# MechaCritter/Python-Visual-Similarity

Hardware: AMD Instinct MI355X
Metric: images/sec encoded + top-k retrieved, VLAD K256 RootSIFT (higher is better)
Workload: dtype f32

## Files before the change

include/pvsim.h:

```cpp
#ifndef PVSIM_H
#define PVSIM_H

#include <stddef.h>
#include <stdint.h>

#ifdef __cplusplus
extern "C" {
#endif

#define PVS_VERSION 103

typedef enum {
  PVS_OK = 0,
  PVS_ERR_INVALID = 1,
  PVS_ERR_NO_DEVICE = 2,
  PVS_ERR_OOM = 3,
  PVS_ERR_UNSUPPORTED = 4,
  PVS_ERR_DIM = 5,
  PVS_ERR_CAPACITY = 6
} pvs_status;

typedef enum {
  PVS_DESC_F32 = 0,
  PVS_DESC_F32_ROOTSIFT = 1,
  PVS_DESC_U8_ROOTSIFT = 2
} pvs_desc_kind;

typedef enum {
  PVS_OPT_ASSIGN_PREFILTER = 0,
  PVS_OPT_VLAD_PATH = 1,
  PVS_OPT_TOPK_SELECT_ONLY = 2,
  PVS_OPT_AGG_VARIANT = 3,
  PVS_OPT_FISHER_SCALE = 4,
  PVS_OPT_COUNT_ = 5
} pvs_option;

typedef struct pvs_ctx pvs_ctx;
typedef struct pvs_codebook pvs_codebook;
typedef struct pvs_gmm pvs_gmm;
typedef struct pvs_pca pvs_pca;
typedef struct pvs_comm pvs_comm;

typedef struct {
  double power_norm_weight;
  double norm_order;
  double epsilon;
} pvs_norm_params;

int pvs_version(void);
// ... 129 lines not shown
  PVS_DSIFT_F32_RAW = 2,
  PVS_DSIFT_F32_QUANT = 3
} pvs_dsift_out;
int pvs_dsift_count(int H, int W, int step, const int32_t* sizes, int n_sizes, int64_t* count);
int pvs_dsift_frames(int H, int W, int step, const int32_t* sizes, int n_sizes, float* frames , int64_t capacity);
int pvs_dsift_dev(pvs_ctx* ctx, const void* d_pixels, int pixel_kind, const int32_t* h_hw, const int64_t* h_pix_offsets,
                  int64_t n_images, int step, const int32_t* sizes, int n_sizes, double contrast_threshold, int out_kind,
                  void* d_out, int64_t out_rows, int64_t* d_row_offsets);

int pvs_sift_workspace(int H, int W, int n_octave_layers, int upsample, size_t* bytes, int64_t* max_rows);
int pvs_sift_dev(pvs_ctx* ctx, const void* d_pixels, int pixel_kind, const int32_t* h_hw, const int64_t* h_pix_offsets,
                 int64_t n_images, int nfeatures, int n_octave_layers, double contrast_threshold, double edge_threshold, double sigma,
                 int upsample, int out_kind, void* d_rows, int64_t capacity_rows, float* d_frames ,
                 int64_t* d_row_offsets, int64_t* h_total_rows);

#define PVS_TIMER_SLOTS 8
int pvs_timers_enable(pvs_ctx* ctx, int on);
int pvs_timers_reset(pvs_ctx* ctx);
int pvs_timers_read(pvs_ctx* ctx, int which, double* total_ms, int64_t* launches);

#ifdef __cplusplus
}
#endif
#endif
```

python-visual-similarity_amd/csrc/api.hip:

```cpp
#include <algorithm>
#include <cmath>
#include <limits>
#include <memory>

#include "common.hpp"

namespace pvs {

static thread_local char g_err[512] = "";

void set_error(const char* fmt, ...) {
  va_list ap;
  va_start(ap, fmt);
  vsnprintf(g_err, sizeof(g_err), fmt, ap);
  va_end(ap);
}

int ws_reserve(pvs_ctx* ctx, int which, size_t bytes, void** out) {
  if (bytes == 0) bytes = 16;
  if (ctx->ws_bytes[which] < bytes) {
    if (ctx->ws[which]) {
      PVS_HIP(hipStreamSynchronize(ctx->stream));
      PVS_HIP(hipFree(ctx->ws[which]));
      ctx->ws[which] = nullptr;
// ... 176 lines not shown

PVS_EXPORT void* pvs_stream(pvs_ctx* ctx) { return ctx ? static_cast<void*>(ctx->stream) : nullptr; }

PVS_EXPORT int pvs_device_name(pvs_ctx* ctx, char* buf, size_t buflen) {
  PVS_NEED(ctx, "ctx");
  PVS_NEED(buf, "buf");
  hipDeviceProp_t prop;
  PVS_HIP(hipGetDeviceProperties(&prop, ctx->device));
  snprintf(buf, buflen, "%s (%s, %d CUs)", prop.name, prop.gcnArchName, prop.multiProcessorCount);
  return PVS_OK;
}

PVS_EXPORT int pvs_set_option(pvs_ctx* ctx, int option, int value) {
  PVS_NEED(ctx, "ctx");
  if (option < 0 || option >= PVS_OPT_COUNT_) PVS_FAIL(PVS_ERR_INVALID, "unknown option %d", option);
  const int hi = option == PVS_OPT_ASSIGN_PREFILTER ? 4 : (option == PVS_OPT_VLAD_PATH || option == PVS_OPT_TOPK_SELECT_ONLY) ? 3 : ((option == PVS_OPT_AGG_VARIANT || option == PVS_OPT_FISHER_SCALE) ? 2 : 1);
  if (value < 0 || value > hi) PVS_FAIL(PVS_ERR_INVALID, "option %d: value %d out of range 0..%d", option, value, hi);
  ctx->opt[option] = value;
  return PVS_OK;
}
PVS_EXPORT int pvs_get_option(pvs_ctx* ctx, int option, int* value) {
  PVS_NEED(ctx, "ctx");
  PVS_NEED(value, "value");
  if (option < 0 || option >= PVS_OPT_COUNT_) PVS_FAIL(PVS_ERR_INVALID, "unknown option %d", option);
  *value = ctx->opt[option];
  return PVS_OK;
}

PVS_EXPORT int pvs_malloc(pvs_ctx* ctx, size_t bytes, void** dptr) {
  PVS_NEED(ctx, "ctx");
  PVS_NEED(dptr, "dptr");
// ... 594 lines not shown
      const int64_t cn = std::min(NC, N - c0);
      const float* iq = d_inv_q ? d_inv_q + q0 : nullptr;
      const float* idb = d_inv_db ? d_inv_db + c0 : nullptr;
      if (f16)
        PVS_TRY(launch_cosine_f16(ctx, q + (size_t)q0 * L * esz, qn, db + (size_t)c0 * L * esz, cn, L, iq, idb, panel, cn));
      else
        PVS_TRY(launch_cosine_f32(ctx, reinterpret_cast<const float*>(q) + q0 * L, qn,
                                  reinterpret_cast<const float*>(db) + c0 * L, cn, L, iq, idb, panel, cn));
      PVS_TRY(launch_topk(ctx, panel, qn, cn, cn, k, col_offset + c0, (merge || c0 > 0) ? 1 : 0, d_idx + q0 * k,
                          d_val + q0 * k));
    }
  }
  return PVS_OK;
}

PVS_EXPORT int pvs_cosine_topk_dev(pvs_ctx* ctx, const float* d_Q, int64_t nq, const float* d_DB, int64_t N, int64_t L,
                                   const float* d_inv_q, const float* d_inv_db, int k, int64_t col_offset, int merge,
                                   int64_t* d_idx, float* d_val) {
  return cosine_topk_impl(ctx, d_Q, nq, d_DB, N, L, false, d_inv_q, d_inv_db, k, col_offset, merge, d_idx, d_val);
}

namespace pvs {
int cosine_topk_exact(pvs_ctx* ctx, const float* d_Q, int64_t nq, const float* d_DB, int64_t N, int64_t L, const float* d_inv_q,
                      const float* d_inv_db, int k, int64_t* d_idx, float* d_val) {
  return cosine_topk_impl(ctx, d_Q, nq, d_DB, N, L, false, d_inv_q, d_inv_db, k, 0, 0, d_idx, d_val);
}
}

PVS_EXPORT int pvs_cosine_topk_filtered_dev(pvs_ctx* ctx, const float* d_Q, int64_t nq, const float* d_DB, int64_t N, int64_t L,
                                            const float* d_inv_q, const float* d_inv_db, int k, int64_t* d_idx, float* d_val,
                                            int64_t* h_stats) {
  PVS_NEED(ctx, "ctx");
  if (h_stats) h_stats[0] = h_stats[1] = h_stats[2] = h_stats[3] = 0;
  if (nq <= 0) return PVS_OK;
  PVS_NEED(d_Q, "Q");
  PVS_NEED(d_idx, "idx");
  PVS_NEED(d_val, "val");
  PVS_HIP(hipSetDevice(ctx->device));
  if (N > 0 && d_DB != nullptr) {
    const int rc = launch_cosine_topk_filtered(ctx, d_Q, nq, d_DB, N, L, d_inv_q, d_inv_db, k, 0, d_idx, d_val, h_stats);
    if (rc != PVS_ERR_UNSUPPORTED) return rc;
    if (h_stats) h_stats[0] = h_stats[1] = h_stats[2] = h_stats[3] = 0;
  }
  return cosine_topk_impl(ctx, d_Q, nq, d_DB, N, L, false, d_inv_q, d_inv_db, k, 0, 0, d_idx, d_val);
}

PVS_EXPORT int pvs_cosine_topk_f16_dev(pvs_ctx* ctx, const void* d_Q16, int64_t nq, const void* d_DB16, int64_t N,
                                       int64_t L, const float* d_inv_q, const float* d_inv_db, int k, int64_t col_offset,
                                       int merge, int64_t* d_idx, float* d_val) {
  return cosine_topk_impl(ctx, d_Q16, nq, d_DB16, N, L, true, d_inv_q, d_inv_db, k, col_offset, merge, d_idx, d_val);
}

PVS_EXPORT int pvs_f32_to_f16_dev(pvs_ctx* ctx, const float* d_src, int64_t n, void* d_dst) {
  PVS_NEED(ctx, "ctx");
  if (n <= 0) return PVS_OK;
// ... 32 lines not shown
  char* d_s = nullptr;
  PVS_TRY(ws_reserve(ctx, 0, q_bytes + (same ? 0 : db_bytes), reinterpret_cast<void**>(&d_in)));
  const size_t nrm = ((size_t)(nq + N) * 4 + 255) / 256 * 256, idxb = ((size_t)nq * k * 8 + 255) / 256 * 256;
  PVS_TRY(ws_reserve(ctx, 1, nrm + idxb + (size_t)nq * k * 4, reinterpret_cast<void**>(&d_s)));
  float* dq = reinterpret_cast<float*>(d_in);
  float* ddb = same ? dq : reinterpret_cast<float*>(d_in + q_bytes);
  PVS_HIP(hipMemcpyAsync(dq, Q, (size_t)nq * L * 4, hipMemcpyHostToDevice, ctx->stream));
  if (!same) PVS_HIP(hipMemcpyAsync(ddb, DB, (size_t)N * L * 4, hipMemcpyHostToDevice, ctx->stream));
  float* invq = reinterpret_cast<float*>(d_s);
  float* invd = invq + nq;
  int64_t* d_idx = reinterpret_cast<int64_t*>(d_s + nrm);
  float* d_val = reinterpret_cast<float*>(d_s + nrm + idxb);
  PVS_TRY(launch_row_inv_norms(ctx, dq, nq, L, invq));
  PVS_TRY(launch_row_inv_norms(ctx, ddb, N, L, invd));
  const float* invd_use = same ? invq : invd;
  if (nq >= 512) PVS_TRY(pvs_cosine_topk_filtered_dev(ctx, dq, nq, ddb, N, L, invq, invd_use, k, d_idx, d_val, nullptr));
  else PVS_TRY(pvs_cosine_topk_dev(ctx, dq, nq, ddb, N, L, invq, invd_use, k, 0, 0, d_idx, d_val));
  PVS_HIP(hipMemcpyAsync(out_idx, d_idx, (size_t)nq * k * 8, hipMemcpyDeviceToHost, ctx->stream));
  PVS_HIP(hipMemcpyAsync(out_val, d_val, (size_t)nq * k * 4, hipMemcpyDeviceToHost, ctx->stream));
  PVS_HIP(hipStreamSynchronize(ctx->stream));
  return PVS_OK;
}


PVS_EXPORT int pvs_row_inv_norms_f64_dev(pvs_ctx* ctx, const double* d_x, int64_t rows, int64_t L, double* d_inv) {
  PVS_NEED(ctx, "ctx");
  if (rows <= 0) return PVS_OK;
  PVS_NEED(d_x, "x");
  PVS_NEED(d_inv, "inv");
  PVS_HIP(hipSetDevice(ctx->device));
  return launch_row_inv_norms_f64(ctx, d_x, rows, L, d_inv);
}
// ... 311 lines not shown
```

python-visual-similarity_amd/csrc/common.hpp:

```cpp
#pragma once
#include <hip/hip_runtime.h>

#include <cmath>
#include <cstdarg>
#include <cstdint>
#include <cstdio>
#include <cstring>
#include <map>
#include <vector>

#include "../../include/pvsim.h"
#include "../../include/pvsim_diag.h"

#define PVS_EXPORT extern "C" __attribute__((visibility("default")))

namespace pvs {

void set_error(const char* fmt, ...);

#define PVS_FAIL(code, ...)        \
  do {                             \
    ::pvs::set_error(__VA_ARGS__); \
    return (code);                 \
  } while (0)
// ... 4 lines not shown
    if (e__ != hipSuccess) {                                                             \
      ::pvs::set_error("%s failed: %s (%s:%d)", #expr, hipGetErrorString(e__), __FILE__, \
                       __LINE__);                                                        \
      return e__ == hipErrorOutOfMemory ? PVS_ERR_OOM : PVS_ERR_NO_DEVICE;               \
    }                                                                                    \
  } while (0)

#define PVS_TRY(expr)                 \
  do {                                \
    int s__ = (expr);                 \
    if (s__ != PVS_OK) return s__;    \
  } while (0)

constexpr int WAVE = 64;

enum TimerSlot { T_ASSIGN = 0, T_AGGREGATE = 1, T_GEMM = 2, T_TOPK = 3, T_FPOST = 4, T_FMOM = 5, T_MISC = 6, T_RESCORE = 7 };

struct TimerRec {
  hipEvent_t a, b;
  int slot;
};

}

struct pvs_ctx {
  int device = 0;
  hipStream_t stream = nullptr;
  bool owns_stream = false;
  int num_cu = 256;
  static constexpr int NWS = 13;
  void* ws[NWS] = {};
  size_t ws_bytes[NWS] = {};
  struct GemmPlanSlot {
    int key[4] = {-1, -1, -1, -1};
    int n_main = 0, n_tail = 0, splitk = 1;
    void* d_tiles = nullptr;
    size_t cap = 0;
  } gemm_plan[5];
  std::map<const void*, int> lds_attr;
  int opt[PVS_OPT_COUNT_] = {1, 0, 0, 0, 0};
  unsigned int* d_queue = nullptr;
  unsigned long long* d_fused_stamps = nullptr;
  bool timers_on = false;
  std::vector<pvs::TimerRec> pending;
  std::vector<hipEvent_t> event_pool;
  std::multimap<size_t, void*> block_cache;
  std::map<void*, size_t> block_size;
  size_t block_cache_bytes = 0;
  void* h_stage = nullptr;
  size_t h_stage_bytes = 0;
  static constexpr int DSIFT_RING = 4;
  void* dsift_h[DSIFT_RING] = {};
  size_t dsift_h_bytes[DSIFT_RING] = {};
  hipEvent_t dsift_ev[DSIFT_RING] = {};
  int dsift_next = 0;
// ... 96 lines not shown
                          const int64_t* d_offsets, int64_t n_images, const int32_t* d_labels,
                          const pvs_norm_params& prm, float* d_out, float* d_inv_norm, bool raw = false,
                          const float2* rowstat = nullptr, int64_t total_hint = 0);
bool vlad_fused_eligible(const pvs_codebook* cb, const void* d_desc, int kind, int ld, const float* d_out);
int launch_vlad_fused(pvs_ctx* ctx, const pvs_codebook* cb, const void* d_desc, int kind, int ld, const int64_t* d_offsets,
                      int64_t n_images, const pvs_norm_params& prm, float* d_out, int32_t* d_labels, float* d_inv_norm, bool raw = false);
int launch_row_inv_norms(pvs_ctx* ctx, const float* d_x, int64_t rows, int64_t L, float* d_inv);
int launch_cosine_f32(pvs_ctx* ctx, const float* A, int64_t M, const float* B, int64_t N, int64_t L,
                      const float* inva, const float* invb, float* out, int64_t ldo);
int launch_cosine_f32_dual(pvs_ctx* ctx, const float* A, int64_t M, const float* B, int64_t N, int64_t L, const float* inva,
                           const float* invb, float* out, int64_t ldo, float* out_t, int64_t ldt);
int launch_cosine_f16(pvs_ctx* ctx, const void* A, int64_t M, const void* B, int64_t N, int64_t L, const float* inva,
                      const float* invb, float* out, int64_t ldo);
int launch_f32_to_f16(pvs_ctx* ctx, const float* src, int64_t n, void* dst);
int launch_cosine_f16_bounded(pvs_ctx* ctx, const void* A, int64_t M, const void* B, int64_t N, int64_t L, const float* inva,
                              const float* invb, float* out, int64_t ldo);
int cosine_topk_exact(pvs_ctx* ctx, const float* d_Q, int64_t nq, const float* d_DB, int64_t N, int64_t L, const float* d_inv_q,
                      const float* d_inv_db, int k, int64_t* d_idx, float* d_val);
int launch_cosine_topk_filtered(pvs_ctx* ctx, const float* Q, int64_t nq, const float* DB, int64_t N, int64_t L,
                                const float* invq, const float* invdb, int k, int64_t col_offset, int64_t* d_idx, float* d_val,
                                int64_t* h_stats);
int launch_cosine_f64(pvs_ctx* ctx, const double* A, int64_t M, const double* B, int64_t N, int64_t L, double* out);
int launch_row_inv_norms_f64(pvs_ctx* ctx, const double* d_x, int64_t rows, int64_t L, double* d_inv);
int launch_cosine_f64_dev(pvs_ctx* ctx, const double* A, int64_t M, const double* B, int64_t N, int64_t L, const double* inva,
                          const double* invb, double* out, int64_t ldo);
bool cosine_dense_rows_eligible(const float* Q, const float* DB, int64_t nq, int64_t L);
int launch_cosine_dense_rows(pvs_ctx* ctx, const float* Q, int64_t nq, const float* DB, int64_t N, int64_t L, const float* invq,
                             const float* invdb, float* scores, int64_t ld);
int launch_topk(pvs_ctx* ctx, const float* scores, int64_t nq, int64_t ncols, int64_t ld, int k,
                int64_t col_offset, int merge, int64_t* d_idx, float* d_val);
int launch_topk_merge(pvs_ctx* ctx, const int64_t* idx_lists, const float* val_lists, int n_lists, int64_t nq,
                      int k, int64_t* d_idx, float* d_val);
int launch_rank_f64(pvs_ctx* ctx, const double* scores, int64_t nq, int64_t ncols, int64_t ld, int k, int64_t* d_idx, double* d_val);
int launch_pca(pvs_ctx* ctx, const pvs_pca* p, const void* d_desc, int kind, int64_t total, float* d_out);
int launch_gmm_posterior(pvs_ctx* ctx, const pvs_gmm* g, const void* d_desc, int kind, int ld, int64_t total,
                         double* d_resp);
// ... 19 lines not shown
```

python-visual-similarity_amd/csrc/cosine.hip:

```cpp
#include <algorithm>
#include <type_traits>

#include "common.hpp"
#include "gemm_mfma.hpp"
#include "gemm_f64.hpp"
#include "gemm_f16_8ph.hpp"
#include "gemm_f16_2lvl.hpp"

namespace pvs {

__device__ __attribute__((aligned(16))) float g_zero16[4] = {0.f, 0.f, 0.f, 0.f};

__global__ __launch_bounds__(256) void row_inv_norms_kernel(const float* __restrict__ x, int64_t rows, int64_t L,
                                                            float* __restrict__ inv, int vec) {
  const int lane = threadIdx.x & 63;
  const int64_t row = (int64_t)blockIdx.x * 4 + (threadIdx.x >> 6);
  if (row >= rows) return;
  const float* p = x + row * L;
  float s0 = 0.f, s1 = 0.f, s2 = 0.f, s3 = 0.f;
  if (vec) {
    const float4* p4 = reinterpret_cast<const float4*>(p);
    for (int64_t i = lane; i < (L >> 2); i += 64) {
      const float4 v = p4[i];
      s0 = fmaf(v.x, v.x, s0); s1 = fmaf(v.y, v.y, s1); s2 = fmaf(v.z, v.z, s2); s3 = fmaf(v.w, v.w, s3);
// ... 15 lines not shown
  PVS_HIP(hipGetLastError());
  return PVS_OK;
}

using GemmMain = GemmCfg<128, 128, 2, 2, 2, false>;
using GemmHalf = GemmCfg<256, 256, 2, 4, 2, true>;
using GemmPre = GemmCfg<128, 128, 2, 2, 2, true>;
template <int MODEL> struct GemmModel;
template <> struct GemmModel<0> { using Cfg = GemmMain; static constexpr bool F16 = false, TWO = true; static constexpr int BM = 128, WN = 2, PER_CU = 2; };
template <> struct GemmModel<1> { using Cfg = GemmHalf; static constexpr bool F16 = true, TWO = false; static constexpr int BM = 256, WN = 4, PER_CU = 1; };
template <> struct GemmModel<2> { using Cfg = GemmPre; static constexpr bool F16 = true, TWO = true; static constexpr int BM = 128, WN = 2, PER_CU = 2; };

using GemmPlan = pvs_ctx::GemmPlanSlot;

static int build_plan(pvs_ctx* ctx, int which, int tiles_m, int tiles_n, bool symm, int slots, GemmPlan** out) {
  GemmPlan& P = ctx->gemm_plan[which];
  const int key[4] = {tiles_m, tiles_n, symm ? 1 : 0, slots};
  if (memcmp(P.key, key, sizeof(key)) != 0) {
    std::vector<GemmTile> t;
    if (symm) {
      const int TS = (tiles_m + 7) / 8;
      for (int si = 0; si < TS; ++si)
        for (int sj = si; sj < TS; ++sj)
          for (int w = 0; w < 64; ++w) {
            const int tm = si * 8 + (w & 7), tn = sj * 8 + (w >> 3);
            if (tm < tiles_m && tn < tiles_m && tn >= tm) t.push_back({tm, tn});
          }
    } else {
      for (int g0 = 0; g0 < tiles_m; g0 += 8) {
        const int gsz = std::min(8, tiles_m - g0);
        for (int tn = 0; tn < tiles_n; ++tn)
          for (int dm = 0; dm < gsz; ++dm) t.push_back({g0 + dm, tn});
// ... 149 lines not shown
  PVS_HIP(hipGetLastError());
  return PVS_OK;
}

int launch_cosine_f16(pvs_ctx* ctx, const void* A, int64_t M, const void* B, int64_t N, int64_t L, const float* inva,
                      const float* invb, float* out, int64_t ldo) {
  if (M <= 0 || N <= 0) return PVS_OK;
  if (L <= 0 || L % 8 != 0 || reinterpret_cast<uintptr_t>(A) % 16 || reinterpret_cast<uintptr_t>(B) % 16)
    PVS_FAIL(PVS_ERR_UNSUPPORTED, "fp16 cosine needs 16-B aligned rows (L %% 8 == 0), got L = %lld", (long long)L);
  if (L > (int64_t)8 * 1024 * 1024) PVS_FAIL(PVS_ERR_UNSUPPORTED, "fp16 cosine: L too large");
  ScopedTimer tm(ctx, T_GEMM);
  return cosine_mfma<1>(ctx, A, M, B, N, L, inva, invb, out, ldo);
}

int launch_cosine_f16_bounded(pvs_ctx* ctx, const void* A, int64_t M, const void* B, int64_t N, int64_t L, const float* inva,
                              const float* invb, float* out, int64_t ldo) {
  if (M <= 0 || N <= 0) return PVS_OK;
  if (L <= 0 || L % 8 != 0 || reinterpret_cast<uintptr_t>(A) % 16 || reinterpret_cast<uintptr_t>(B) % 16)
    PVS_FAIL(PVS_ERR_UNSUPPORTED, "fp16 cosine needs 16-B aligned rows (L %% 8 == 0), got L = %lld", (long long)L);
  ScopedTimer tm(ctx, T_GEMM);
  constexpr int64_t SEG = 32768;
  const char* a = static_cast<const char*>(A);
  const char* b = static_cast<const char*>(B);
  for (int64_t k0 = 0; k0 < L; k0 += SEG)
    PVS_TRY(cosine_mfma<2>(ctx, a + k0 * 2, M, A == B ? a + k0 * 2 : b + k0 * 2, N, std::min(SEG, L - k0), inva, invb, out, ldo, nullptr, 0, L,
                           k0 > 0 ? 1 : 0));
  return PVS_OK;
}

template <typename T>
__global__ __launch_bounds__(256) void cosine_gemm_generic_kernel(const T* __restrict__ A, int64_t M,
                                                                  const T* __restrict__ B, int64_t N, int64_t L,
                                                                  const T* __restrict__ inva,
                                                                  const T* __restrict__ invb, T* __restrict__ out,
                                                                  int64_t ldo) {
// ... 155 lines not shown
```

python-visual-similarity_amd/csrc/filter.hip:

```cpp
#include <algorithm>
#include <cmath>
#include <vector>

#include "common.hpp"

namespace pvs {

constexpr int FLT_PASS = 16;
constexpr int FLT_SK = 32;
constexpr int FLT_THREADS = FLT_PASS * 32;

static double filter_eps(int64_t L) {
  return 9.77e-4 * (1.0 + 1.0 / 4096.0) + (1088.0 + (double)L / 1024.0 + 2.0 * (double)((L + 32767) / 32768)) * 1.1920929e-7 +
         2.98e-8 * std::sqrt((double)L);
}

__global__ __launch_bounds__(256) void filter_rows_to_f16_kernel(const float* __restrict__ x, int64_t rows, int64_t L,
                                                                 const float* __restrict__ inv_in, _Float16* __restrict__ out,
                                                                 float* __restrict__ inv_out, unsigned long long* __restrict__ stats) {
  __shared__ float red[4];
  __shared__ int bad[4];
  const int64_t row = blockIdx.x;
  const float4* xr = reinterpret_cast<const float4*>(x + row * L);
  const int64_t n4 = L / 4;
// ... 31 lines not shown
    inv_out[row] = (inv_in ? inv_in[row] : 1.f) * ldexpf(1.f, -sh);
    if (nf) atomicAdd(&stats[0], 1ull);
  }
}

__global__ __launch_bounds__(256) void filter_collect_kernel(const float* __restrict__ S, int64_t nq, int64_t ncols, int64_t ld,
                                                             const int64_t* __restrict__ aidx, const float* __restrict__ aval,
                                                             int k, float margin, int cap, int64_t col_offset, int first,
                                                             int64_t* __restrict__ cand_idx, int* __restrict__ count,
                                                             unsigned long long* __restrict__ stats) {
  const int lane = threadIdx.x & 63;
  const int64_t q = (int64_t)blockIdx.x * 4 + (threadIdx.x >> 6);
  if (q >= nq) return;
  const bool full = aidx[q * k + k - 1] >= 0;
  const float thr = full ? aval[q * k + k - 1] - margin : -INFINITY;
  int base = first ? 0 : count[q];
  const int base0 = base;
  for (int64_t c0 = 0; c0 < ncols; c0 += 64) {
    const int64_t c = c0 + lane;
    const bool pred = c < ncols && S[q * ld + c] >= thr;
    const unsigned long long mask = __ballot(pred);
    if (pred) {
      const int slot = base + __popcll(mask & ((1ull << lane) - 1ull));
      if (slot < cap) cand_idx[((int64_t)(slot / k) * nq + q) * k + slot % k] = col_offset + c;
    }
    base += __popcll(mask);
  }
  if (lane == 0) {
    count[q] = base;
    atomicAdd(&stats[2], (unsigned long long)(base - base0));
    if (base > cap && base0 <= cap) atomicAdd(&stats[1], 1ull);
  }
}

struct RescoreArgs {
  const float* Q;
  const float* DB;
  int64_t nq, L;
  const float* invq;
  const float* invdb;
  const int64_t* cand_idx;
  float* cand_val;
  const int* count;
  int cap, k;
  int64_t col_offset;
// ... 113 lines not shown
int launch_cosine_dense_rows(pvs_ctx* ctx, const float* Q, int64_t nq, const float* DB, int64_t N, int64_t L, const float* invq,
                             const float* invdb, float* scores, int64_t ld) {
  if (!cosine_dense_rows_eligible(Q, DB, nq, L)) PVS_FAIL(PVS_ERR_UNSUPPORTED, "dense row scoring: shape does not qualify");
  if (N <= 0) return PVS_OK;
  const int64_t groups = (N + FLT_PASS - 1) / FLT_PASS;
  if (groups > 0x7fffffffLL) PVS_FAIL(PVS_ERR_UNSUPPORTED, "dense row scoring: too many rows");
  RescoreArgs ra{Q, DB, nq, L, invq, invdb, nullptr, scores, nullptr, 0, 1, 0, N, ld};
  ScopedTimer tm(ctx, T_GEMM);
  hipLaunchKernelGGL(filter_rescore_kernel<true>, dim3((unsigned)groups, (unsigned)nq), dim3(FLT_THREADS), 0, ctx->stream, ra);
  PVS_HIP(hipGetLastError());
  return PVS_OK;
}

int launch_cosine_topk_filtered(pvs_ctx* ctx, const float* Q, int64_t nq, const float* DB, int64_t N, int64_t L,
                                const float* invq, const float* invdb, int k, int64_t col_offset, int64_t* d_idx, float* d_val,
                                int64_t* h_stats) {
  if (col_offset != 0) PVS_FAIL(PVS_ERR_UNSUPPORTED, "filtered top-k: col_offset must be 0");
  if (nq <= 0 || N <= 0) PVS_FAIL(PVS_ERR_UNSUPPORTED, "filtered top-k: empty input");
  if (L > (int64_t)8 * 1024 * 1024) PVS_FAIL(PVS_ERR_UNSUPPORTED, "filtered top-k: rows too long");
  if (L % 8 != 0 || L < 8 || reinterpret_cast<uintptr_t>(Q) % 16 || reinterpret_cast<uintptr_t>(DB) % 16)
    PVS_FAIL(PVS_ERR_UNSUPPORTED, "filtered top-k needs 16-B aligned rows with L %% 8 == 0");
  if (k < 1 || k > 128) PVS_FAIL(PVS_ERR_UNSUPPORTED, "filtered top-k: k <= 128");
  const int64_t NC = std::min<int64_t>(N, 32768);
  const bool multi = N > NC;
  const bool same = (Q == DB) && (nq == N) && (invq == invdb);
  const bool square = same && !multi && (int64_t)nq * N <= ((int64_t)1 << 28);
  const int cap_lists = ((multi ? 16 : 4) * k + (multi ? 128 : 64) + k - 1) / k;
  const int cap = cap_lists * k;
  const int64_t QT = square ? nq : std::min<int64_t>(nq, std::max<int64_t>(256, ((int64_t)1 << 28) / NC));
  const double eps = filter_eps(L);
  const float margin = (float)(2.0 * eps);

  const size_t q16_b = ((size_t)nq * L * 2 + 255) / 256 * 256, db16_b = same ? 0 : ((size_t)N * L * 2 + 255) / 256 * 256;
  char* w5 = nullptr;
  if (ws_reserve(ctx, 5, q16_b + db16_b, reinterpret_cast<void**>(&w5)) != PVS_OK) {
    (void)hipGetLastError();
    PVS_FAIL(PVS_ERR_UNSUPPORTED, "filtered top-k: no device memory for the fp16 copies (%zu bytes)", q16_b + db16_b);
  }
  _Float16* q16 = reinterpret_cast<_Float16*>(w5);
  _Float16* db16 = same ? q16 : reinterpret_cast<_Float16*>(w5 + q16_b);
  auto al = [](size_t b) { return (b + 255) / 256 * 256; };
  const size_t o_invq = 0, o_invd = o_invq + al((size_t)nq * 4), o_stats = o_invd + al((size_t)N * 4),
               o_aidx = o_stats + 256, o_aval = o_aidx + al((size_t)QT * k * 8), o_cidx = o_aval + al((size_t)QT * k * 4),
               o_cval = o_cidx + al((size_t)QT * cap * 8), o_cnt = o_cval + al((size_t)QT * cap * 4), o_end = o_cnt + al((size_t)QT * 4);
  char* w6 = nullptr;
  PVS_TRY(ws_reserve(ctx, 6, o_end, reinterpret_cast<void**>(&w6)));
  float* invq16 = reinterpret_cast<float*>(w6 + o_invq);
  float* invd16 = same ? invq16 : reinterpret_cast<float*>(w6 + o_invd);
  unsigned long long* stats = reinterpret_cast<unsigned long long*>(w6 + o_stats);
  int64_t* aidx = reinterpret_cast<int64_t*>(w6 + o_aidx);
  float* aval = reinterpret_cast<float*>(w6 + o_aval);
  int64_t* cidx = reinterpret_cast<int64_t*>(w6 + o_cidx);
  float* cval = reinterpret_cast<float*>(w6 + o_cval);
  int* cnt = reinterpret_cast<int*>(w6 + o_cnt);
  float* panel = nullptr;
  PVS_TRY(ws_reserve(ctx, 2, (size_t)QT * NC * sizeof(float), reinterpret_cast<void**>(&panel)));
  PVS_HIP(hipMemsetAsync(stats, 0, 32, ctx->stream));

  {
    ScopedTimer tm(ctx, T_MISC);
    hipLaunchKernelGGL(filter_rows_to_f16_kernel, dim3((unsigned)nq), dim3(256), 0, ctx->stream, Q, nq, L, invq, q16, invq16, stats);
    if (!same)
      hipLaunchKernelGGL(filter_rows_to_f16_kernel, dim3((unsigned)N), dim3(256), 0, ctx->stream, DB, N, L, invdb, db16, invd16, stats);
    PVS_HIP(hipGetLastError());
  }
  unsigned long long hs[4] = {0, 0, 0, 0};
  PVS_HIP(hipMemcpyAsync(hs, stats, 8, hipMemcpyDeviceToHost, ctx->stream));
  PVS_HIP(hipStreamSynchronize(ctx->stream));
  if (hs[0]) PVS_FAIL(PVS_ERR_UNSUPPORTED, "filtered top-k: %llu rows hold non-finite values or an extreme dynamic range", hs[0]);

  std::vector<int> h_cnt;
  for (int64_t q0 = 0; q0 < nq; q0 += QT) {
    const int64_t qn = std::min(QT, nq - q0);
    PVS_TRY(ws_reserve(ctx, 2, (size_t)QT * NC * sizeof(float), reinterpret_cast<void**>(&panel)));
    PVS_HIP(hipMemsetAsync(cidx, 0xff, (size_t)qn * cap * 8, ctx->stream));
    for (int64_t c0 = 0; c0 < N; c0 += NC) {
      const int64_t cn = std::min(NC, N - c0);
      PVS_TRY(launch_cosine_f16_bounded(ctx, q16 + q0 * L, qn, db16 + c0 * L, cn, L, invq16 + q0, invd16 + c0, panel, cn));
      PVS_TRY(launch_topk(ctx, panel, qn, cn, cn, k, c0, c0 > 0 ? 1 : 0, aidx, aval));
      ScopedTimer tm(ctx, T_TOPK);
      hipLaunchKernelGGL(filter_collect_kernel, dim3((unsigned)((qn + 3) / 4)), dim3(256), 0, ctx->stream, panel, qn, cn, cn, aidx, aval, k,
                         margin, cap, c0, c0 == 0 ? 1 : 0, cidx, cnt, stats);
    }
    PVS_HIP(hipMemcpyAsync(hs, stats, 24, hipMemcpyDeviceToHost, ctx->stream));
    PVS_HIP(hipStreamSynchronize(ctx->stream));
    if (hs[1] * 10 > (unsigned long long)qn) PVS_FAIL(PVS_ERR_UNSUPPORTED, "filtered top-k: %llu of %lld queries exceed the candidate slots", hs[1], (long long)qn);
    {
      ScopedTimer tm(ctx, T_RESCORE);
      RescoreArgs ra{Q + q0 * L, DB, qn, L, invq ? invq + q0 : nullptr, invdb, cidx, cval, cnt, cap, k, 0};
      hipLaunchKernelGGL(filter_rescore_kernel<false>, dim3((unsigned)qn), dim3(FLT_THREADS), 0, ctx->stream, ra);
    }
    PVS_HIP(hipGetLastError());
    PVS_TRY(launch_topk_merge(ctx, cidx, cval, cap_lists, qn, k, d_idx + q0 * k, d_val + q0 * k));
    PVS_HIP(hipMemcpyAsync(hs, stats, 24, hipMemcpyDeviceToHost, ctx->stream));
    PVS_HIP(hipStreamSynchronize(ctx->stream));
    if (hs[1]) {
      h_cnt.resize((size_t)qn);
      PVS_HIP(hipMemcpy(h_cnt.data(), cnt, (size_t)qn * 4, hipMemcpyDeviceToHost));
      std::vector<int64_t> rows;
      for (int64_t i = 0; i < qn; ++i)
        if (h_cnt[(size_t)i] > cap) rows.push_back(i);
      const int64_t nr = (int64_t)rows.size();
      const int64_t rb = std::max<int64_t>(1, std::min<int64_t>(nr, ((int64_t)1 << 28) / N));
      char* w4 = nullptr;
      const size_t rows_b = al((size_t)nr * 8), g_b = al((size_t)rb * L * 4), gi_b = al((size_t)rb * 4), li_b = al((size_t)rb * k * 8);
      PVS_TRY(ws_reserve(ctx, 3, rows_b + g_b + gi_b + li_b + al((size_t)rb * k * 4), reinterpret_cast<void**>(&w4)));
      int64_t* d_rows = reinterpret_cast<int64_t*>(w4);
      float* gq = reinterpret_cast<float*>(w4 + rows_b);
      float* gi = reinterpret_cast<float*>(w4 + rows_b + g_b);
      int64_t* li = reinterpret_cast<int64_t*>(w4 + rows_b + g_b + gi_b);
      float* lv = reinterpret_cast<float*>(w4 + rows_b + g_b + gi_b + li_b);
      PVS_HIP(hipMemcpyAsync(d_rows, rows.data(), (size_t)nr * 8, hipMemcpyHostToDevice, ctx->stream));
      for (int64_t r0 = 0; r0 < nr; r0 += rb) {
        const int64_t rn = std::min(rb, nr - r0);
        hipLaunchKernelGGL(filter_gather_rows_kernel, dim3((unsigned)rn), dim3(256), 0, ctx->stream, Q + q0 * L, d_rows + r0, L, gq,
                           invq ? invq + q0 : nullptr, gi);
        PVS_HIP(hipGetLastError());
        PVS_TRY(cosine_topk_exact(ctx, gq, rn, DB, N, L, gi, invdb, k, li, lv));
        hipLaunchKernelGGL(filter_scatter_lists_kernel, dim3((unsigned)rn), dim3(64), 0, ctx->stream, li, lv, d_rows + r0, k,
                           d_idx + q0 * k, d_val + q0 * k);
      }
// ... 13 lines not shown
```

python-visual-similarity_amd/pvsim/_ffi.py:

```python
from __future__ import annotations

import ctypes as C
import os
import threading

import numpy as np

from ._errors import CapacityError

_HERE = os.path.dirname(os.path.abspath(__file__))
LIB_PATH = os.environ.get("PVSIM_LIB", os.path.join(_HERE, "libpvsim_hip.so"))

PVS_OK, PVS_ERR_INVALID, PVS_ERR_NO_DEVICE, PVS_ERR_OOM, PVS_ERR_UNSUPPORTED, PVS_ERR_DIM, PVS_ERR_CAPACITY = range(7)
_EXC = {PVS_ERR_INVALID: ValueError, PVS_ERR_NO_DEVICE: RuntimeError, PVS_ERR_OOM: MemoryError,
        PVS_ERR_UNSUPPORTED: NotImplementedError, PVS_ERR_DIM: RuntimeError, PVS_ERR_CAPACITY: CapacityError}

DESC_F32, DESC_F32_ROOTSIFT, DESC_U8_ROOTSIFT = 0, 1, 2
OPT_ASSIGN_PREFILTER, OPT_VLAD_PATH, OPT_TOPK_SELECT_ONLY, OPT_AGG_VARIANT, OPT_FISHER_SCALE = 0, 1, 2, 3, 4
PIX_U8_RGB, PIX_U8_GRAY, PIX_F32_RGB, PIX_F32_GRAY = 0, 1, 2, 3
DSIFT_U8, DSIFT_F32, DSIFT_F32_RAW, DSIFT_F32_QUANT = 0, 1, 2, 3
VLAD_PATH_AUTO, VLAD_PATH_GATHER, VLAD_PATH_STREAM, VLAD_PATH_FUSED = 0, 1, 2, 3
TIMER_NAMES = ("assign", "aggregate", "cosine_gemm", "topk", "fisher_posterior", "fisher_moments", "misc", "rescore")


class NormParams(C.Structure):
    _fields_ = [("power_norm_weight", C.c_double), ("norm_order", C.c_double), ("epsilon", C.c_double)]


_vp, _i64, _int, _sz = C.c_void_p, C.c_int64, C.c_int, C.c_size_t
_pp = C.POINTER(C.c_void_p)
_np = C.POINTER(NormParams)

SIGNATURES = {
    "pvs_version": [],
    "pvs_last_error": [],
    "pvs_device_count": [C.POINTER(C.c_int)],
    "pvs_init": [_int, _vp, _pp],
# ... 151 lines not shown
```

python-visual-similarity_amd/pvsim/distributed.py:

```python
from __future__ import annotations

import ctypes as C
import socket
import struct
import time
from typing import Callable

import numpy as np

__all__ = ["shard_range", "gather_blocks", "mask_padding", "retrieve_sharded", "device_score_block",
           "retrieve_symmetric", "symmetric_local", "symmetric_finish", "DeviceOps", "ShardedVLADIndex",
           "DevArray", "DevicePool", "RcclComm", "new_unique_id", "exchange_unique_id"]

_ITEM = {"float32": 4, "int64": 8, "int32": 4, "float64": 8, "float16": 2, "uint8": 1}


def shard_range(n_total: int, world: int, rank: int) -> tuple[int, int, int]:
    block = (n_total + world - 1) // world
    lo = min(n_total, rank * block)
    return lo, min(n_total, lo + block), block


def exchange_chunks(n_total: int, world: int, n_chunks: int):
    _, _, block = shard_range(n_total, world, 0)
# ... 290 lines not shown

    def score(q, n_q, db, n_db, inv_q, inv_db, k, col_offset, merge, idx, val):
        ctx.cosine_topk_dev(q.data_ptr(), n_q, db.data_ptr(), n_db, q.shape[1], inv_q.data_ptr(), inv_db.data_ptr(),
                            k, col_offset, merge, idx.data_ptr(), val.data_ptr())

    return score


class DeviceOps:

    def __init__(self, ctx, same_stream: bool = False):
        self.ctx = ctx
        self.same_stream = same_stream

    def sym_topk(self, q, n, inv, k, col_offset, idx, val):
        self.ctx.cosine_topk_dev(q.data_ptr(), n, q.data_ptr(), n, q.shape[1], inv.data_ptr(), inv.data_ptr(), k,
                                 col_offset, False, idx.data_ptr(), val.data_ptr())

    def dual(self, a, m, b, n, inv_a, inv_b, panel, panel_t):
        self.ctx.cosine_dual_dev(a.data_ptr(), m, b.data_ptr(), n, a.shape[1], inv_a.data_ptr(), inv_b.data_ptr(),
                                 panel.data_ptr(), n, panel_t.data_ptr(), m)

    def topk(self, scores, nq, ncols, k, col_offset, merge, idx, val):
        self.ctx.topk_dev(scores.data_ptr(), nq, ncols, ncols, k, col_offset, merge, idx.data_ptr(), val.data_ptr())

    def merge(self, idx_lists, val_lists, n_lists, nq, k, idx, val):
        self.ctx.topk_merge_dev(idx_lists.data_ptr(), val_lists.data_ptr(), n_lists, nq, k, idx.data_ptr(), val.data_ptr())

    def sync(self):
        if not self.same_stream:
            self.ctx.sync()

# ... 177 lines not shown
```

Before: 420,700.

## Route default cosine top-k through the filtered fp16 prefilter path with probing

pvs_cosine_topk_dev now defaults to the fp16 prefilter + exact rescore path for large query/database sizes. Before committing to the full run it probes on the first 256 rows. The gemm plan cache becomes two-way so the probe and main tile shapes do not evict each other. A per-tile stats sync moves into the prefilter step, and NaN thresholds now force the overflow path. The aim is to avoid full fp32 GEMM plus top-k for most candidates, at the cost of extra syncs and a fallback risk when candidate slots overflow.

```diff
diff --git a/include/pvsim.h b/include/pvsim.h
--- a/include/pvsim.h
+++ b/include/pvsim.h
@@ -32,7 +32,8 @@
   PVS_OPT_TOPK_SELECT_ONLY = 2,
   PVS_OPT_AGG_VARIANT = 3,
   PVS_OPT_FISHER_SCALE = 4,
-  PVS_OPT_COUNT_ = 5
+  PVS_OPT_TOPK_PATH = 5,
+  PVS_OPT_COUNT_ = 6
 } pvs_option;
 
 typedef struct pvs_ctx pvs_ctx;
@@ -192,7 +193,7 @@
                  int upsample, int out_kind, void* d_rows, int64_t capacity_rows, float* d_frames ,
                  int64_t* d_row_offsets, int64_t* h_total_rows);
 
-#define PVS_TIMER_SLOTS 8
+#define PVS_TIMER_SLOTS 9
 int pvs_timers_enable(pvs_ctx* ctx, int on);
 int pvs_timers_reset(pvs_ctx* ctx);
 int pvs_timers_read(pvs_ctx* ctx, int which, double* total_ms, int64_t* launches);
diff --git a/python-visual-similarity_amd/csrc/api.hip b/python-visual-similarity_amd/csrc/api.hip
--- a/python-visual-similarity_amd/csrc/api.hip
+++ b/python-visual-similarity_amd/csrc/api.hip
@@ -214,7 +214,7 @@
 PVS_EXPORT int pvs_set_option(pvs_ctx* ctx, int option, int value) {
   PVS_NEED(ctx, "ctx");
   if (option < 0 || option >= PVS_OPT_COUNT_) PVS_FAIL(PVS_ERR_INVALID, "unknown option %d", option);
-  const int hi = option == PVS_OPT_ASSIGN_PREFILTER ? 4 : (option == PVS_OPT_VLAD_PATH || option == PVS_OPT_TOPK_SELECT_ONLY) ? 3 : ((option == PVS_OPT_AGG_VARIANT || option == PVS_OPT_FISHER_SCALE) ? 2 : 1);
+  const int hi = option == PVS_OPT_ASSIGN_PREFILTER ? 4 : (option == PVS_OPT_VLAD_PATH || option == PVS_OPT_TOPK_SELECT_ONLY) ? 3 : ((option == PVS_OPT_AGG_VARIANT || option == PVS_OPT_FISHER_SCALE || option == PVS_OPT_TOPK_PATH) ? 2 : 1);
   if (value < 0 || value > hi) PVS_FAIL(PVS_ERR_INVALID, "option %d: value %d out of range 0..%d", option, value, hi);
   ctx->opt[option] = value;
   return PVS_OK;
@@ -839,9 +839,24 @@
   return PVS_OK;
 }
 
+constexpr int64_t TOPK_FILTER_MIN_NQ = 512;
+static int topk_filter_mode(const pvs_ctx* ctx, int64_t nq, int64_t N, int64_t col_offset, int merge) {
+  const int opt = ctx->opt[PVS_OPT_TOPK_PATH];
+  if (opt == 1 || col_offset != 0 || merge != 0 || nq <= 0 || N <= 0) return 0;
+  if (opt == 2) return 2;
+  return (nq >= TOPK_FILTER_MIN_NQ && N >= TOPK_FILTER_MIN_NQ) ? 1 : 0;
+}
+
 PVS_EXPORT int pvs_cosine_topk_dev(pvs_ctx* ctx, const float* d_Q, int64_t nq, const float* d_DB, int64_t N, int64_t L,
                                    const float* d_inv_q, const float* d_inv_db, int k, int64_t col_offset, int merge,
                                    int64_t* d_idx, float* d_val) {
+  PVS_NEED(ctx, "ctx");
+  const int mode = topk_filter_mode(ctx, nq, N, col_offset, merge);
+  if (mode != 0 && d_Q != nullptr && d_DB != nullptr && d_idx != nullptr && d_val != nullptr) {
+    PVS_HIP(hipSetDevice(ctx->device));
+    const int rc = launch_cosine_topk_filtered(ctx, d_Q, nq, d_DB, N, L, d_inv_q, d_inv_db, k, 0, d_idx, d_val, nullptr, mode == 1);
+    if (rc != PVS_ERR_UNSUPPORTED) return rc;
+  }
   return cosine_topk_impl(ctx, d_Q, nq, d_DB, N, L, false, d_inv_q, d_inv_db, k, col_offset, merge, d_idx, d_val);
 }
 
@@ -863,7 +878,7 @@
   PVS_NEED(d_val, "val");
   PVS_HIP(hipSetDevice(ctx->device));
   if (N > 0 && d_DB != nullptr) {
-    const int rc = launch_cosine_topk_filtered(ctx, d_Q, nq, d_DB, N, L, d_inv_q, d_inv_db, k, 0, d_idx, d_val, h_stats);
+    const int rc = launch_cosine_topk_filtered(ctx, d_Q, nq, d_DB, N, L, d_inv_q, d_inv_db, k, 0, d_idx, d_val, h_stats, false);
     if (rc != PVS_ERR_UNSUPPORTED) return rc;
     if (h_stats) h_stats[0] = h_stats[1] = h_stats[2] = h_stats[3] = 0;
   }
@@ -926,8 +941,7 @@
   PVS_TRY(launch_row_inv_norms(ctx, dq, nq, L, invq));
   PVS_TRY(launch_row_inv_norms(ctx, ddb, N, L, invd));
   const float* invd_use = same ? invq : invd;
-  if (nq >= 512) PVS_TRY(pvs_cosine_topk_filtered_dev(ctx, dq, nq, ddb, N, L, invq, invd_use, k, d_idx, d_val, nullptr));
-  else PVS_TRY(pvs_cosine_topk_dev(ctx, dq, nq, ddb, N, L, invq, invd_use, k, 0, 0, d_idx, d_val));
+  PVS_TRY(pvs_cosine_topk_dev(ctx, dq, nq, ddb, N, L, invq, invd_use, k, 0, 0, d_idx, d_val));
   PVS_HIP(hipMemcpyAsync(out_idx, d_idx, (size_t)nq * k * 8, hipMemcpyDeviceToHost, ctx->stream));
   PVS_HIP(hipMemcpyAsync(out_val, d_val, (size_t)nq * k * 4, hipMemcpyDeviceToHost, ctx->stream));
   PVS_HIP(hipStreamSynchronize(ctx->stream));
diff --git a/python-visual-similarity_amd/csrc/common.hpp b/python-visual-similarity_amd/csrc/common.hpp
--- a/python-visual-similarity_amd/csrc/common.hpp
+++ b/python-visual-similarity_amd/csrc/common.hpp
@@ -42,7 +42,7 @@
 
 constexpr int WAVE = 64;
 
-enum TimerSlot { T_ASSIGN = 0, T_AGGREGATE = 1, T_GEMM = 2, T_TOPK = 3, T_FPOST = 4, T_FMOM = 5, T_MISC = 6, T_RESCORE = 7 };
+enum TimerSlot { T_ASSIGN = 0, T_AGGREGATE = 1, T_GEMM = 2, T_TOPK = 3, T_FPOST = 4, T_FMOM = 5, T_MISC = 6, T_RESCORE = 7, T_PROBE = 8 };
 
 struct TimerRec {
   hipEvent_t a, b;
@@ -64,9 +64,10 @@
     int n_main = 0, n_tail = 0, splitk = 1;
     void* d_tiles = nullptr;
     size_t cap = 0;
-  } gemm_plan[5];
+  } gemm_plan[10];
+  int gemm_plan_last[5] = {0, 0, 0, 0, 0};
   std::map<const void*, int> lds_attr;
-  int opt[PVS_OPT_COUNT_] = {1, 0, 0, 0, 0};
+  int opt[PVS_OPT_COUNT_] = {1, 0, 0, 0, 0, 0};
   unsigned int* d_queue = nullptr;
   unsigned long long* d_fused_stamps = nullptr;
   bool timers_on = false;
@@ -193,12 +194,12 @@
                       const float* invb, float* out, int64_t ldo);
 int launch_f32_to_f16(pvs_ctx* ctx, const float* src, int64_t n, void* dst);
 int launch_cosine_f16_bounded(pvs_ctx* ctx, const void* A, int64_t M, const void* B, int64_t N, int64_t L, const float* inva,
-                              const float* invb, float* out, int64_t ldo);
+                              const float* invb, float* out, int64_t ldo, int timer_slot = T_GEMM);
 int cosine_topk_exact(pvs_ctx* ctx, const float* d_Q, int64_t nq, const float* d_DB, int64_t N, int64_t L, const float* d_inv_q,
                       const float* d_inv_db, int k, int64_t* d_idx, float* d_val);
 int launch_cosine_topk_filtered(pvs_ctx* ctx, const float* Q, int64_t nq, const float* DB, int64_t N, int64_t L,
                                 const float* invq, const float* invdb, int k, int64_t col_offset, int64_t* d_idx, float* d_val,
-                                int64_t* h_stats);
+                                int64_t* h_stats, bool probe);
 int launch_cosine_f64(pvs_ctx* ctx, const double* A, int64_t M, const double* B, int64_t N, int64_t L, double* out);
 int launch_row_inv_norms_f64(pvs_ctx* ctx, const double* d_x, int64_t rows, int64_t L, double* d_inv);
 int launch_cosine_f64_dev(pvs_ctx* ctx, const double* A, int64_t M, const double* B, int64_t N, int64_t L, const double* inva,
diff --git a/python-visual-similarity_amd/csrc/cosine.hip b/python-visual-similarity_amd/csrc/cosine.hip
--- a/python-visual-similarity_amd/csrc/cosine.hip
+++ b/python-visual-similarity_amd/csrc/cosine.hip
@@ -53,8 +53,11 @@
 using GemmPlan = pvs_ctx::GemmPlanSlot;
 
 static int build_plan(pvs_ctx* ctx, int which, int tiles_m, int tiles_n, bool symm, int slots, GemmPlan** out) {
-  GemmPlan& P = ctx->gemm_plan[which];
   const int key[4] = {tiles_m, tiles_n, symm ? 1 : 0, slots};
+  int way = ctx->gemm_plan_last[which];
+  if (memcmp(ctx->gemm_plan[2 * which + way].key, key, sizeof(key)) != 0) way ^= 1;
+  ctx->gemm_plan_last[which] = way;
+  GemmPlan& P = ctx->gemm_plan[2 * which + way];
   if (memcmp(P.key, key, sizeof(key)) != 0) {
     std::vector<GemmTile> t;
     if (symm) {
@@ -234,11 +237,11 @@
 }
 
 int launch_cosine_f16_bounded(pvs_ctx* ctx, const void* A, int64_t M, const void* B, int64_t N, int64_t L, const float* inva,
-                              const float* invb, float* out, int64_t ldo) {
+                              const float* invb, float* out, int64_t ldo, int timer_slot) {
   if (M <= 0 || N <= 0) return PVS_OK;
   if (L <= 0 || L % 8 != 0 || reinterpret_cast<uintptr_t>(A) % 16 || reinterpret_cast<uintptr_t>(B) % 16)
     PVS_FAIL(PVS_ERR_UNSUPPORTED, "fp16 cosine needs 16-B aligned rows (L %% 8 == 0), got L = %lld", (long long)L);
-  ScopedTimer tm(ctx, T_GEMM);
+  ScopedTimer tm(ctx, timer_slot);
   constexpr int64_t SEG = 32768;
   const char* a = static_cast<const char*>(A);
   const char* b = static_cast<const char*>(B);
diff --git a/python-visual-similarity_amd/csrc/filter.hip b/python-visual-similarity_amd/csrc/filter.hip
--- a/python-visual-similarity_amd/csrc/filter.hip
+++ b/python-visual-similarity_amd/csrc/filter.hip
@@ -69,6 +69,7 @@
   if (q >= nq) return;
   const bool full = aidx[q * k + k - 1] >= 0;
   const float thr = full ? aval[q * k + k - 1] - margin : -INFINITY;
+  const bool nan_kth = thr != thr;
   int base = first ? 0 : count[q];
   const int base0 = base;
   for (int64_t c0 = 0; c0 < ncols; c0 += 64) {
@@ -82,8 +83,9 @@
     base += __popcll(mask);
   }
   if (lane == 0) {
+    atomicAdd(&stats[2], (unsigned long long)(base - base0));
+    if (nan_kth && base <= cap) base = cap + 1;
     count[q] = base;
-    atomicAdd(&stats[2], (unsigned long long)(base - base0));
     if (base > cap && base0 <= cap) atomicAdd(&stats[1], 1ull);
   }
 }
@@ -227,7 +229,7 @@
 
 int launch_cosine_topk_filtered(pvs_ctx* ctx, const float* Q, int64_t nq, const float* DB, int64_t N, int64_t L,
                                 const float* invq, const float* invdb, int k, int64_t col_offset, int64_t* d_idx, float* d_val,
-                                int64_t* h_stats) {
+                                int64_t* h_stats, bool probe) {
   if (col_offset != 0) PVS_FAIL(PVS_ERR_UNSUPPORTED, "filtered top-k: col_offset must be 0");
   if (nq <= 0 || N <= 0) PVS_FAIL(PVS_ERR_UNSUPPORTED, "filtered top-k: empty input");
   if (L > (int64_t)8 * 1024 * 1024) PVS_FAIL(PVS_ERR_UNSUPPORTED, "filtered top-k: rows too long");
@@ -256,8 +258,16 @@
   const size_t o_invq = 0, o_invd = o_invq + al((size_t)nq * 4), o_stats = o_invd + al((size_t)N * 4),
                o_aidx = o_stats + 256, o_aval = o_aidx + al((size_t)QT * k * 8), o_cidx = o_aval + al((size_t)QT * k * 4),
                o_cval = o_cidx + al((size_t)QT * cap * 8), o_cnt = o_cval + al((size_t)QT * cap * 4), o_end = o_cnt + al((size_t)QT * 4);
+  auto reserve = [&](int slot, size_t bytes, void** out) -> int {
+    const int rc = ws_reserve(ctx, slot, bytes, out);
+    if (rc == PVS_ERR_OOM) {
+      (void)hipGetLastError();
+      PVS_FAIL(PVS_ERR_UNSUPPORTED, "filtered top-k: no device memory for workspace %d (%zu bytes)", slot, bytes);
+    }
+    return rc;
+  };
   char* w6 = nullptr;
-  PVS_TRY(ws_reserve(ctx, 6, o_end, reinterpret_cast<void**>(&w6)));
+  PVS_TRY(reserve(6, o_end, reinterpret_cast<void**>(&w6)));
   float* invq16 = reinterpret_cast<float*>(w6 + o_invq);
   float* invd16 = same ? invq16 : reinterpret_cast<float*>(w6 + o_invd);
   unsigned long long* stats = reinterpret_cast<unsigned long long*>(w6 + o_stats);
@@ -267,7 +277,7 @@
   float* cval = reinterpret_cast<float*>(w6 + o_cval);
   int* cnt = reinterpret_cast<int*>(w6 + o_cnt);
   float* panel = nullptr;
-  PVS_TRY(ws_reserve(ctx, 2, (size_t)QT * NC * sizeof(float), reinterpret_cast<void**>(&panel)));
+  PVS_TRY(reserve(2, (size_t)QT * NC * sizeof(float), reinterpret_cast<void**>(&panel)));
   PVS_HIP(hipMemsetAsync(stats, 0, 32, ctx->stream));
 
   {
@@ -278,26 +288,35 @@
     PVS_HIP(hipGetLastError());
   }
   unsigned long long hs[4] = {0, 0, 0, 0};
-  PVS_HIP(hipMemcpyAsync(hs, stats, 8, hipMemcpyDeviceToHost, ctx->stream));
-  PVS_HIP(hipStreamSynchronize(ctx->stream));
-  if (hs[0]) PVS_FAIL(PVS_ERR_UNSUPPORTED, "filtered top-k: %llu rows hold non-finite values or an extreme dynamic range", hs[0]);
-
-  std::vector<int> h_cnt;
-  for (int64_t q0 = 0; q0 < nq; q0 += QT) {
-    const int64_t qn = std::min(QT, nq - q0);
-    PVS_TRY(ws_reserve(ctx, 2, (size_t)QT * NC * sizeof(float), reinterpret_cast<void**>(&panel)));
+  auto prefilter_rows = [&](int64_t q0, int64_t qn, int gemm_slot) -> int {
+    PVS_TRY(reserve(2, (size_t)QT * NC * sizeof(float), reinterpret_cast<void**>(&panel)));
     PVS_HIP(hipMemsetAsync(cidx, 0xff, (size_t)qn * cap * 8, ctx->stream));
     for (int64_t c0 = 0; c0 < N; c0 += NC) {
       const int64_t cn = std::min(NC, N - c0);
-      PVS_TRY(launch_cosine_f16_bounded(ctx, q16 + q0 * L, qn, db16 + c0 * L, cn, L, invq16 + q0, invd16 + c0, panel, cn));
+      PVS_TRY(launch_cosine_f16_bounded(ctx, q16 + q0 * L, qn, db16 + c0 * L, cn, L, invq16 + q0, invd16 + c0, panel, cn, gemm_slot));
       PVS_TRY(launch_topk(ctx, panel, qn, cn, cn, k, c0, c0 > 0 ? 1 : 0, aidx, aval));
       ScopedTimer tm(ctx, T_TOPK);
       hipLaunchKernelGGL(filter_collect_kernel, dim3((unsigned)((qn + 3) / 4)), dim3(256), 0, ctx->stream, panel, qn, cn, cn, aidx, aval, k,
                          margin, cap, c0, c0 == 0 ? 1 : 0, cidx, cnt, stats);
     }
+    PVS_HIP(hipGetLastError());
     PVS_HIP(hipMemcpyAsync(hs, stats, 24, hipMemcpyDeviceToHost, ctx->stream));
     PVS_HIP(hipStreamSynchronize(ctx->stream));
+    if (hs[0]) PVS_FAIL(PVS_ERR_UNSUPPORTED, "filtered top-k: %llu rows hold non-finite values or an extreme dynamic range", hs[0]);
     if (hs[1] * 10 > (unsigned long long)qn) PVS_FAIL(PVS_ERR_UNSUPPORTED, "filtered top-k: %llu of %lld queries exceed the candidate slots", hs[1], (long long)qn);
+    return PVS_OK;
+  };
+
+  constexpr int64_t FLT_PROBE_ROWS = 256;
+  if (probe && nq > 2 * FLT_PROBE_ROWS) {
+    PVS_TRY(prefilter_rows(0, FLT_PROBE_ROWS, T_PROBE));
+    PVS_HIP(hipMemsetAsync(stats + 1, 0, 16, ctx->stream));
+  }
+
+  std::vector<int> h_cnt;
+  for (int64_t q0 = 0; q0 < nq; q0 += QT) {
+    const int64_t qn = std::min(QT, nq - q0);
+    PVS_TRY(prefilter_rows(q0, qn, T_GEMM));
     {
       ScopedTimer tm(ctx, T_RESCORE);
       RescoreArgs ra{Q + q0 * L, DB, qn, L, invq ? invq + q0 : nullptr, invdb, cidx, cval, cnt, cap, k, 0};
@@ -305,8 +324,6 @@
     }
     PVS_HIP(hipGetLastError());
     PVS_TRY(launch_topk_merge(ctx, cidx, cval, cap_lists, qn, k, d_idx + q0 * k, d_val + q0 * k));
-    PVS_HIP(hipMemcpyAsync(hs, stats, 24, hipMemcpyDeviceToHost, ctx->stream));
-    PVS_HIP(hipStreamSynchronize(ctx->stream));
     if (hs[1]) {
       h_cnt.resize((size_t)qn);
       PVS_HIP(hipMemcpy(h_cnt.data(), cnt, (size_t)qn * 4, hipMemcpyDeviceToHost));
@@ -317,7 +334,7 @@
       const int64_t rb = std::max<int64_t>(1, std::min<int64_t>(nr, ((int64_t)1 << 28) / N));
       char* w4 = nullptr;
       const size_t rows_b = al((size_t)nr * 8), g_b = al((size_t)rb * L * 4), gi_b = al((size_t)rb * 4), li_b = al((size_t)rb * k * 8);
-      PVS_TRY(ws_reserve(ctx, 3, rows_b + g_b + gi_b + li_b + al((size_t)rb * k * 4), reinterpret_cast<void**>(&w4)));
+      PVS_TRY(reserve(3, rows_b + g_b + gi_b + li_b + al((size_t)rb * k * 4), reinterpret_cast<void**>(&w4)));
       int64_t* d_rows = reinterpret_cast<int64_t*>(w4);
       float* gq = reinterpret_cast<float*>(w4 + rows_b);
       float* gi = reinterpret_cast<float*>(w4 + rows_b + g_b);
diff --git a/python-visual-similarity_amd/pvsim/_ffi.py b/python-visual-similarity_amd/pvsim/_ffi.py
--- a/python-visual-similarity_amd/pvsim/_ffi.py
+++ b/python-visual-similarity_amd/pvsim/_ffi.py
@@ -17,10 +17,11 @@
 
 DESC_F32, DESC_F32_ROOTSIFT, DESC_U8_ROOTSIFT = 0, 1, 2
 OPT_ASSIGN_PREFILTER, OPT_VLAD_PATH, OPT_TOPK_SELECT_ONLY, OPT_AGG_VARIANT, OPT_FISHER_SCALE = 0, 1, 2, 3, 4
+OPT_TOPK_PATH = 5
 PIX_U8_RGB, PIX_U8_GRAY, PIX_F32_RGB, PIX_F32_GRAY = 0, 1, 2, 3
 DSIFT_U8, DSIFT_F32, DSIFT_F32_RAW, DSIFT_F32_QUANT = 0, 1, 2, 3
 VLAD_PATH_AUTO, VLAD_PATH_GATHER, VLAD_PATH_STREAM, VLAD_PATH_FUSED = 0, 1, 2, 3
-TIMER_NAMES = ("assign", "aggregate", "cosine_gemm", "topk", "fisher_posterior", "fisher_moments", "misc", "rescore")
+TIMER_NAMES = ("assign", "aggregate", "cosine_gemm", "topk", "fisher_posterior", "fisher_moments", "misc", "rescore", "probe")
 
 
 class NormParams(C.Structure):
diff --git a/python-visual-similarity_amd/pvsim/distributed.py b/python-visual-similarity_amd/pvsim/distributed.py
--- a/python-visual-similarity_amd/pvsim/distributed.py
+++ b/python-visual-similarity_amd/pvsim/distributed.py
@@ -7,6 +7,8 @@
 from typing import Callable
 
 import numpy as np
+
+from . import _ffi
 
 __all__ = ["shard_range", "gather_blocks", "mask_padding", "retrieve_sharded", "device_score_block",
            "retrieve_symmetric", "symmetric_local", "symmetric_finish", "DeviceOps", "ShardedVLADIndex",
@@ -328,8 +330,9 @@
         self.same_stream = same_stream
 
     def sym_topk(self, q, n, inv, k, col_offset, idx, val):
-        self.ctx.cosine_topk_dev(q.data_ptr(), n, q.data_ptr(), n, q.shape[1], inv.data_ptr(), inv.data_ptr(), k,
-                                 col_offset, False, idx.data_ptr(), val.data_ptr())
+        with self.ctx.option(_ffi.OPT_TOPK_PATH, 1):
+            self.ctx.cosine_topk_dev(q.data_ptr(), n, q.data_ptr(), n, q.shape[1], inv.data_ptr(), inv.data_ptr(), k,
+                                     col_offset, False, idx.data_ptr(), val.data_ptr())
 
     def dual(self, a, m, b, n, inv_a, inv_b, panel, panel_t):
         self.ctx.cosine_dual_dev(a.data_ptr(), m, b.data_ptr(), n, a.shape[1], inv_a.data_ptr(), inv_b.data_ptr(),
```

After: 909,600, median of 6. 2.16x the previous value.
